# tingyu215/VACNIC

Measured on AMD Instinct MI355X. Metric: train samples/sec, BART-large + CLIP ViT-L/14 full VACNIC step, GoodNews-shaped batch, higher is better.
Workload: dtype bf16

## Files before the change

vacnic_amd/csrc/gemm.hip:

```cpp
#include "gemm_kernel.h"
#include <vector>

using namespace vacgemm;

namespace {

#define VAC_BFLY(ACC, LANE, OFF, HALF)                                                 \
  {                                                                              \
    const bool up = ((LANE) & OFF) != 0;                                           \
    _Pragma("unroll") for (int i = 0; i < HALF; ++i) {                           \
      const float send = up ? ACC[i] : ACC[HALF + i];                            \
      const float keep = up ? ACC[HALF + i] : ACC[i];                            \
      ACC[i] = keep + __shfl_xor(send, OFF, 64);                                 \
    }                                                                            \
  }
#define VAC_BFLY32(ACC, LANE, V, IDX)                                                                                     \
  VAC_BFLY(ACC, LANE, 32, 16) VAC_BFLY(ACC, LANE, 16, 8) VAC_BFLY(ACC, LANE, 8, 4) VAC_BFLY(ACC, LANE, 4, 2) VAC_BFLY(ACC, LANE, 2, 1) \
  float V = ACC[0] + __shfl_xor(ACC[0], 1, 64);                                                                       \
  const int IDX = ((((LANE) >> 5) & 1) << 4) | ((((LANE) >> 4) & 1) << 3) | ((((LANE) >> 3) & 1) << 2) | ((((LANE) >> 2) & 1) << 1) | (((LANE) >> 1) & 1);

template <int MR, int CW, int KW>
__global__ __launch_bounds__(64 * KW) void gemm_skinny_kernel(GemmP p) {
  const int lane = threadIdx.x & 63;
  const int kw = KW == 1 ? 0 : __builtin_amdgcn_readfirstlane(threadIdx.x >> 6);
// ... 208 lines not shown
static const double kFixedUnits = 27e6;

static double cfg_cost(const TileCfg& c, int64_t M, int64_t N, int64_t kper, int64_t z) {
  const int64_t tiles = ((M + c.bm - 1) / c.bm) * ((N + c.bn - 1) / c.bn) * z;
  const int64_t rounds = (tiles + c.slots - 1) / c.slots;
  return (double)rounds * ((double)c.per_cu * c.bm * c.bn * (double)kper / c.eff + kFixedUnits);
}

static int gemm_one(const vacnic_gemm_args* a, int hint, void* stream, int ce_mode = 0, int ce_col0 = 0, bool ce_smooth = false);

static int gemm_env_debug() {
  static int env_debug = -1;
  if (env_debug < 0) { const char* e = getenv("VACNIC_GEMM_DEBUG"); env_debug = e ? atoi(e) : 0; }
  return env_debug;
}

extern "C" int64_t vacnic_gemm_workspace_bytes(int64_t M, int64_t N, int64_t split_k) {
  if (M <= 0 || N <= 0 || split_k <= 1) return 0;
  const int64_t mp = (M + 255) / 256 * 256, np = (N + 255) / 256 * 256;
  return mp * np * 4 * split_k;
}
extern "C" int64_t vacnic_gemm_counters(int64_t M, int64_t N) {
  if (M <= 0 || N <= 0) return 0;
  return ((M + 63) / 64) * ((N + 127) / 128);
}

extern "C" int vacnic_gemm_bf16(const vacnic_gemm_args* a, void* stream) {
  VPLAN_REC_STRUCT(vacnic_gemm_bf16, a, stream);
  VCHECK(a && a->x && a->w && a->out, VACNIC_BAD_SHAPE, "gemm: null operand");
  VCHECK(a->M > 0 && a->N > 0 && a->K > 0, VACNIC_BAD_SHAPE, "gemm: empty problem M=%ld N=%ld K=%ld",
         (long)a->M, (long)a->N, (long)a->K);
  if (a->tile_hint != 0) return gemm_one(a, a->tile_hint, stream);
  if (a->M <= 8 && !a->x_kstrided && !a->w_kstrided && a->split_k <= 1 && !a->preact && !a->dact_src && !a->residual && !a->xsum &&
      (a->K & 7) == 0)
    return gemm_one(a, 8, stream);
  const int split = a->split_k < 1 ? 1 : a->split_k;
  int64_t kper = (a->K + split - 1) / split;
  kper = (kper + BK - 1) / BK * BK;
  const int64_t z = (a->K + kper - 1) / kper;
  int best = 0; double best_cost = 1e300;
  for (int i = 0; i < 3; ++i) {
    if (i == 0 && (a->M < 256 || a->N < 256)) continue;
    const double c = cfg_cost(kCfgs[i], a->M, a->N, kper, z);
    if (c < best_cost) { best_cost = c; best = i; }
  }
  int split_cfg = -1; int64_t m_main = 0; double split_cost = best_cost;
  for (int i = 0; i < 2; ++i) {
    const int64_t rem = a->M % kCfgs[i].bm;
    if (rem == 0 || a->M - rem < kCfgs[i].bm || (i == 0 && a->N < 256)) continue;
    const double c = cfg_cost(kCfgs[i], a->M - rem, a->N, kper, z) + cfg_cost(kCfgs[2], rem, a->N, kper, z);
    if (c < 0.85 * split_cost) { split_cost = c; split_cfg = i; m_main = a->M - rem; }
  }
  const bool fwd8 = !a->x_kstrided && !a->w_kstrided && a->drop_p == 0.f;
  auto loop_of = [&](int hint) { return hint == 256 && fwd8 ? 258 : hint; };
  if (split_cfg < 0) return gemm_one(a, loop_of(kCfgs[best].hint), stream);
  vacnic_gemm_args main_a = *a, tail_a = *a;
  main_a.M = m_main;
  tail_a.M = a->M - m_main;
  const int64_t xoff = a->x_kstrided ? m_main : m_main * a->ldx;
  tail_a.x = (const char*)a->x + xoff * 2;
  const int64_t osz = a->out_mode == 0 ? 2 : 4;
  tail_a.out = (char*)a->out + m_main * a->ldo * osz;
  if (a->preact) tail_a.preact = (char*)a->preact + m_main * a->ldo * 2;
  if (a->dact_src) tail_a.dact_src = (const char*)a->dact_src + m_main * a->ldo * 2;
  if (a->residual) tail_a.residual = (const char*)a->residual + m_main * a->ldo * 2;
  if (a->xsum) tail_a.xsum = a->xsum + m_main;
  if (int e = gemm_one(&main_a, loop_of(kCfgs[split_cfg].hint), stream)) return e;
  return gemm_one(&tail_a, kCfgs[2].hint, stream);
}

static int gemm_one(const vacnic_gemm_args* a, int tile_hint, void* stream, int ce_mode, int ce_col0, bool ce_smooth) {
  VCHECK((a->ldx & 7) == 0 && (a->ldw & 7) == 0, VACNIC_MISALIGNED, "gemm: ldx/ldw must be multiples of 8");
  VCHECK(aligned16(a->x) && aligned16(a->w), VACNIC_MISALIGNED, "gemm: x/w must be 16-byte aligned");
  VCHECK(a->out_mode >= 0 && a->out_mode <= 2, VACNIC_BAD_DTYPE, "gemm: bad out_mode %d", a->out_mode);
  const int split = a->split_k < 1 ? 1 : a->split_k;
  VCHECK(split == 1 || a->out_mode == 2 || a->workspace, VACNIC_UNSUPPORTED, "gemm: split_k needs out_mode 2 or a fix-up workspace");
  if (a->workspace && split > 1) {
    VCHECK(a->counters && aligned16(a->workspace), VACNIC_BAD_SHAPE, "gemm: the split-K fix-up needs `counters` and a 16-byte aligned workspace");
    VCHECK(a->workspace_bytes >= vacnic_gemm_workspace_bytes(a->M, a->N, split) && a->counters_len >= vacnic_gemm_counters(a->M, a->N), VACNIC_BAD_SHAPE,
           "gemm: fix-up workspace %ld B / %ld counters, need %ld B / %ld", (long)a->workspace_bytes, (long)a->counters_len,
           (long)vacnic_gemm_workspace_bytes(a->M, a->N, split), (long)vacnic_gemm_counters(a->M, a->N));
    VCHECK(tile_hint != 8 && !ce_mode, VACNIC_UNSUPPORTED, "gemm: no split-K fix-up in the skinny / cross-entropy kernels");
  }
  VCHECK(a->bias == nullptr || aligned16(a->bias), VACNIC_MISALIGNED, "gemm: bias must be 16-byte aligned");
  VCHECK(a->ldo >= a->N, VACNIC_BAD_SHAPE, "gemm: ldo < N");
  VCHECK(!a->xsum || ce_mode || (a->x_kstrided && a->w_kstrided), VACNIC_UNSUPPORTED,
         "gemm: xsum (row sums of X) is implemented for the weight-gradient layout only (x_kstrided and w_kstrided)");
  if (a->x_kstrided) VCHECK(a->ldx >= ((a->M + 7) & ~7LL), VACNIC_BAD_SHAPE, "gemm: ldx too small for K-strided X");
  else VCHECK(a->ldx >= ((a->K + 7) & ~7LL), VACNIC_BAD_SHAPE, "gemm: ldx < round_up(K, 8) for K-contiguous X");
  if (a->w_kstrided) VCHECK(a->ldw >= ((a->N + 7) & ~7LL), VACNIC_BAD_SHAPE, "gemm: ldw too small for K-strided W");
  else VCHECK(a->ldw >= ((a->K + 7) & ~7LL), VACNIC_BAD_SHAPE, "gemm: ldw < round_up(K, 8) for K-contiguous W");

  auto span = [](int64_t rows, int64_t cols, int64_t ld) { return ((rows - 1) * ld + cols) * 2; };
  const int64_t K8 = (a->K + 7) & ~7LL;
  const int64_t xb = a->x_kstrided ? span(a->K, (a->M + 7) & ~7LL, a->ldx) : span(a->M, K8, a->ldx);
  const int64_t wb = a->w_kstrided ? span(a->K, (a->N + 7) & ~7LL, a->ldw) : span(a->N, K8, a->ldw);
  VCHECK(xb < 0x7ffffff0LL && wb < 0x7ffffff0LL, VACNIC_UNSUPPORTED, "gemm: operand larger than 2 GiB");

  GemmP p;
  p.x = (const bf16_t*)a->x; p.w = (const bf16_t*)a->w; p.bias = a->bias;
  p.out = a->out; p.preact = (bf16_t*)a->preact; p.dact_src = (const bf16_t*)a->dact_src;
  p.residual = (const bf16_t*)a->residual;
  p.xsum = a->xsum;
  p.M = (int)a->M; p.N = (int)a->N; p.K = (int)a->K;
  p.ldx = (int)a->ldx; p.ldw = (int)a->ldw; p.ldo = (int)a->ldo;
  p.act = a->act; p.out_mode = ce_mode ? ce_mode : a->out_mode; p.split_k = split;
  p.ce_col0 = ce_col0;
  int kps = (int)((a->K + split - 1) / split);
  kps = (kps + BK - 1) / BK * BK;
  p.k_per_split = kps;
  const int zsplits = (int)((a->K + kps - 1) / kps);
  p.split_k = zsplits;
  p.alpha = a->alpha;
  p.x_bytes = (unsigned)xb; p.w_bytes = (unsigned)wb;
  p.tiles_m = p.tiles_n = 0;
  p.ws = (a->workspace && zsplits > 1) ? (float*)a->workspace : nullptr;
  p.cnt = p.ws ? a->counters : nullptr;
  p.drop_thr = 0; p.drop_inv = 1.f; p.drop_seed = a->drop_seed; p.drop_seed_dev = (const unsigned long long*)a->drop_seed_dev;
  if (a->drop_p != 0.f) {
    VCHECK(a->drop_p > 0.f && a->drop_p < 1.f, VACNIC_BAD_SHAPE, "gemm: drop_p must be in [0, 1)");
    VCHECK(a->out_mode == 0 && a->ldo == a->N && (a->N & 15) == 0 && !ce_mode && tile_hint != 8, VACNIC_UNSUPPORTED,
           "gemm: fused activation dropout needs a contiguous bf16 output with N %% 16 == 0 (use vacnic_dropout_bf16)");
    VCHECK((zsplits == 1 || p.ws) , VACNIC_UNSUPPORTED, "gemm: fused activation dropout with split-K needs the fix-up workspace");
    unsigned thr = (unsigned)(a->drop_p * 256.f + 0.5f);
    if (thr > 255) thr = 255;
    p.drop_thr = thr;
    p.drop_inv = 256.f / (256.f - (float)thr);
  }
  hipStream_t s = (hipStream_t)stream;
  if (tile_hint == 8) {
    VCHECK(a->M <= 8 && !a->x_kstrided && !a->w_kstrided && zsplits == 1 && !a->preact && !a->dact_src && !a->residual && !a->xsum &&
           (a->K & 7) == 0, VACNIC_UNSUPPORTED, "gemm: the skinny kernel needs M <= 8, K-contiguous operands, K %% 8 == 0 and a plain epilogue");
    constexpr int CW = 4;
    dim3 grid((unsigned)((a->N + CW - 1) / CW));
    if (a->K >= 2048 && a->N <= 8192) hipLaunchKernelGGL((gemm_skinny_kernel<8, CW, 4>), grid, dim3(256), 0, s, p);
    else hipLaunchKernelGGL((gemm_skinny_kernel<8, CW, 1>), grid, dim3(64), 0, s, p);
    VLAUNCH_CHECK();
    return VACNIC_OK;
  }
  const int force = tile_hint % 1000;
  p.debug = tile_hint / 1000 | gemm_env_debug();
  if (((a->M - 1) * a->ldo + a->N) * 2 >= 0x7ffffff0LL) p.debug |= EPI_F32_STAGED;
  if ((a->preact != nullptr) + (a->dact_src != nullptr) + (a->residual != nullptr) > 1) p.debug |= EPI_F32_STAGED;
  if (p.drop_thr && !a->preact && !a->dact_src) p.debug |= EPI_F32_STAGED;
  const bool big = force == 256;
  const bool mid = force == 128;
  if (p.drop_thr) {
    if (big) return launch_t256d(p, a->x_kstrided, a->w_kstrided, zsplits, s);
    if (force == 264) return launch_t264d(p, a->x_kstrided, a->w_kstrided, zsplits, s);
    return launch_t64d(p, a->x_kstrided, a->w_kstrided, zsplits, s);
  }
  if (force == 260) return launch_t260(p, a->x_kstrided, a->w_kstrided, zsplits, s);
  if (force == 261) return launch_t261(p, a->x_kstrided, a->w_kstrided, zsplits, s);
  if (force == 262) return launch_t262(p, a->x_kstrided, a->w_kstrided, zsplits, s);
  if (force == 264) return launch_t264(p, a->x_kstrided, a->w_kstrided, zsplits, s);
  if (force == 258 && !ce_mode) return launch_t258(p, a->x_kstrided, a->w_kstrided, zsplits, s);
  if (ce_mode && ce_smooth) return launch_t256cels(p, a->x_kstrided, a->w_kstrided, zsplits, s);
  if (ce_mode) return launch_t256ce(p, a->x_kstrided, a->w_kstrided, zsplits, s);
  if (big) return launch_t256(p, a->x_kstrided, a->w_kstrided, zsplits, s);
  if (mid) return launch_t128(p, a->x_kstrided, a->w_kstrided, zsplits, s);
  return launch_t64(p, a->x_kstrided, a->w_kstrided, zsplits, s);
}

extern "C" int vacnic_wgrad_group(const vacnic_wgrad_job* jobs, int64_t njobs, void* stream) {
  VCHECK(jobs && njobs > 0, VACNIC_BAD_SHAPE, "wgrad_group: no jobs");
  vplan::Guard vplan_guard__;
  if (vplan::outermost()) {
    std::vector<vacnic_wgrad_job> copy__(jobs, jobs + njobs);
    vplan::push([copy__, stream]() { return vacnic_wgrad_group(copy__.data(), (int64_t)copy__.size(), stream); });
  }
  constexpr int64_t US = (int64_t)GROUP_UT * 128;
  GroupP g;
  g.nunits = 0;
  g.debug = gemm_env_debug() & ~DBG_RETURN;
  auto flush = [&]() -> int {
    if (g.nunits == 0) return VACNIC_OK;
    int kmax = 0;
    for (int i = 0; i < g.nunits; ++i) kmax = g.u[i].K > kmax ? g.u[i].K : kmax;
    g.k_per_phase = (kmax + BK - 1) / BK * BK;
    g.kphase = 0;
    const int e = launch_group128(g, (hipStream_t)stream);
    g.nunits = 0;
    return e;
  };
  auto span = [](int64_t rows, int64_t cols, int64_t ld) { return ((rows - 1) * ld + cols) * 2; };
  for (int64_t j = 0; j < njobs; ++j) {
    const vacnic_wgrad_job& a = jobs[j];
    VCHECK(a.dy && a.x && a.dw, VACNIC_BAD_SHAPE, "wgrad_group: job %ld has a null operand", (long)j);
    VCHECK(a.M > 0 && a.N > 0 && a.K > 0, VACNIC_BAD_SHAPE, "wgrad_group: job %ld is empty (M=%ld N=%ld K=%ld)", (long)j, (long)a.M, (long)a.N, (long)a.K);
    VCHECK((a.lddy & 7) == 0 && (a.ldx & 7) == 0 && aligned16(a.dy) && aligned16(a.x), VACNIC_MISALIGNED,
           "wgrad_group: job %ld: dy / x rows must be 16-byte aligned (ld %% 8 == 0)", (long)j);
    VCHECK(a.lddy >= ((a.N + 7) & ~7LL) && a.ldx >= ((a.K + 7) & ~7LL) && a.lddw >= a.K, VACNIC_BAD_SHAPE,
           "wgrad_group: job %ld: leading dimension too small", (long)j);
    VCHECK((a.lddw & 3) == 0 && aligned16(a.dw), VACNIC_MISALIGNED, "wgrad_group: job %ld: dw rows must be 16-byte aligned", (long)j);
    const int64_t xb = span(a.M, (a.N + 7) & ~7LL, a.lddy), wb = span(a.M, (a.K + 7) & ~7LL, a.ldx);
    VCHECK(xb < 0x7ffffff0LL && wb < 0x7ffffff0LL, VACNIC_UNSUPPORTED, "wgrad_group: job %ld: operand larger than 2 GiB", (long)j);
    for (int64_t um0 = 0; um0 < a.N; um0 += US)
      for (int64_t un0 = 0; un0 < a.K; un0 += US) {
        GroupUnit& u = g.u[g.nunits++];
// ... 175 lines not shown
```

vacnic_amd/csrc/gemm_kernel.h:

```cpp
#pragma once
#include "common.h"
#include <stdlib.h>

namespace vacgemm {


constexpr int BK = 64;
constexpr int OOB = 0x7ffffff0;

struct GemmP {
  const bf16_t* x; const bf16_t* w; const float* bias;
  void* out; bf16_t* preact; const bf16_t* dact_src; const bf16_t* residual;
  float* xsum;
  int M, N, K;
  int ldx, ldw, ldo;
  int act, out_mode, split_k, k_per_split;
  float alpha;
  unsigned x_bytes, w_bytes;
  int tiles_m, tiles_n;
  int ce_col0;
  unsigned drop_thr; float drop_inv; unsigned long long drop_seed; const unsigned long long* drop_seed_dev;
  float* ws;
  unsigned* cnt;
  int debug;
// ... 159 lines not shown
#pragma unroll
    for (int j = 0; j < 8; ++j) v[j] *= act_bwd(p.act, d[j]);
  } else if (p.act != VACNIC_ACT_NONE) {
#pragma unroll
    for (int j = 0; j < 8; ++j) v[j] = act_fwd(p.act, v[j]);
  }
  if (p.residual) {
    float d[8] = {0, 0, 0, 0, 0, 0, 0, 0};
    if (vec) load8bf(p.residual + off, d);
    else for (int j = 0; j < nv; ++j) d[j] = bf2f(p.residual[off + j]);
#pragma unroll
    for (int j = 0; j < 8; ++j) v[j] += d[j];
  }
  if (p.debug & DBG_NO_STORE) {
    if (v[0] == 12345.678f) ((bf16_t*)p.out)[off] = 0;
  } else if (p.out_mode == 0) {
    bf16_t* o = (bf16_t*)p.out + off;
    if (vec) store8bf(o, v);
    else for (int j = 0; j < nv; ++j) o[j] = f2bf(v[j]);
  } else if (p.out_mode == 1) {
    float* o = (float*)p.out + off;
    if (nv == 8 && (p.ldo & 3) == 0) {
      *(f32x4*)o = (f32x4){v[0], v[1], v[2], v[3]};
      *(f32x4*)(o + 4) = (f32x4){v[4], v[5], v[6], v[7]};
    } else {
      for (int j = 0; j < nv; ++j) o[j] = v[j];
    }
  } else {
    float* o = (float*)p.out + off;
    if (nv == 8 && (p.ldo & 3) == 0) {
      f32x4 a0 = *(f32x4*)o, a1 = *(f32x4*)(o + 4);
#pragma unroll
      for (int j = 0; j < 4; ++j) { a0[j] += v[j]; a1[j] += v[4 + j]; }
      *(f32x4*)o = a0; *(f32x4*)(o + 4) = a1;
    } else {
      for (int j = 0; j < nv; ++j) o[j] += v[j];
    }
  }
}

template <int V> struct IC { static constexpr int value = V; };

__device__ __forceinline__ void lds_barrier() {
  asm volatile("s_waitcnt lgkmcnt(0)" ::: "memory");
  __builtin_amdgcn_s_barrier();
  asm volatile("" ::: "memory");
}



template <int N>
__device__ __forceinline__ void wait_vm_lgkm() { asm volatile("s_waitcnt vmcnt(%0) lgkmcnt(0)" ::"n"(N) : "memory"); }

template <int FB, int FA>
__device__ __forceinline__ void p8_loop(f32x4 (&acc)[FB][FA], char* smem, __amdgpu_buffer_rsrc_t xs, __amdgpu_buffer_rsrc_t ws,
                                        int m0, int n0, int RX, int RW, int kbeg, int kend, int ntile, int ldx, int ldw,
                                        int wave, int lane) {
  static_assert(FB == 4 && FA == 8, "128 x 64 outputs per wave");
  constexpr int HALF = 16384, BUF = 4 * HALF;
  constexpr int SLOT_W0 = 0, SLOT_X0 = HALF, SLOT_W1 = 2 * HALF, SLOT_X1 = 3 * HALF;
  const int wm = wave & 1, wn = wave >> 1;
  const int sr = lane >> 2, sc = (lane & 3) ^ (((lane >> 5) & 1) << 1);
  unsigned xoff[2], woff[2];
#pragma unroll
  for (int h = 0; h < 2; ++h) {
    const int gx = m0 + (wave >> 2) * 128 + h * 64 + (wave & 3) * 16 + sr;
    const int gw = n0 + (wave >> 1) * 64 + h * 32 + (wave & 1) * 16 + sr;
    xoff[h] = gx < RX ? ((unsigned)gx * (unsigned)ldx + (unsigned)(sc * 8)) * 2u : (unsigned)OOB;
    woff[h] = gw < RW ? ((unsigned)gw * (unsigned)ldw + (unsigned)(sc * 8)) * 2u : (unsigned)OOB;
  }
  const int klim = kend - sc * 8;
  char* const sdst = smem + wave * 2048;
  auto stage = [&](__amdgpu_buffer_rsrc_t rsrc, unsigned roff, int slot, int t) {
    const int k0 = kbeg + t * 64;
    const unsigned v0 = k0 < klim ? roff + (unsigned)k0 * 2u : (unsigned)OOB;
    const unsigned v1 = k0 + 32 < klim ? roff + (unsigned)(k0 + 32) * 2u : (unsigned)OOB;
    char* d = sdst + slot;
    __builtin_amdgcn_raw_ptr_buffer_load_lds(rsrc, LDS_PTR(d), 16, (int)v0, 0, 0, 0);
    __builtin_amdgcn_raw_ptr_buffer_load_lds(rsrc, LDS_PTR(d + 1024), 16, (int)v1, 0, 0, 0);
  };
  const int fro = (lane & 15) * 64 + (((lane >> 4) ^ (((lane >> 3) & 1) << 1)) << 4);
  const char* const xrd = smem + fro + wm * 8192;
  const char* const wrd = smem + fro + wn * 4096;

  stage(ws, woff[0], SLOT_W0, 0); stage(xs, xoff[0], SLOT_X0, 0); stage(ws, woff[1], SLOT_W1, 0); stage(xs, xoff[1], SLOT_X1, 0);
  stage(ws, woff[0], BUF + SLOT_W0, 1); stage(xs, xoff[0], BUF + SLOT_X0, 1); stage(ws, woff[1], BUF + SLOT_W1, 1);
  asm volatile("s_waitcnt vmcnt(6)" ::: "memory");
  __builtin_amdgcn_sched_barrier(0);
  __builtin_amdgcn_s_barrier();
  __builtin_amdgcn_sched_barrier(0);
  const bool grp_b = wave >= 4;
  if (grp_b) { __builtin_amdgcn_sched_barrier(0); __builtin_amdgcn_s_barrier(); __builtin_amdgcn_sched_barrier(0); }

  bf16x8 xf[4][2], w0[2][2], w1[2][2];
#define VAC_P8_BAR()  __builtin_amdgcn_sched_barrier(0); __builtin_amdgcn_s_barrier(); __builtin_amdgcn_sched_barrier(0)
#define VAC_P8_MFMA(A0, B0, WF)                                                                                          \
  asm volatile("s_waitcnt lgkmcnt(0)" ::: "memory");                                                                     \
  __builtin_amdgcn_sched_barrier(0);                                                                                     \
  __builtin_amdgcn_s_setprio(1);                                                                                         \
  _Pragma("unroll") for (int kk = 0; kk < 2; ++kk)                                                                       \
    _Pragma("unroll") for (int b = 0; b < 2; ++b)                                                                        \
      _Pragma("unroll") for (int a = 0; a < 4; ++a)                                                                      \
        acc[B0 + b][A0 + a] = __builtin_amdgcn_mfma_f32_16x16x32_bf16(WF[b][kk], xf[a][kk], acc[B0 + b][A0 + a], 0, 0, 0); \
  __builtin_amdgcn_s_setprio(0);                                                                                         \
  VAC_P8_BAR()
  auto ktile = [&](auto par_c, int t) {
    constexpr int PAR = decltype(par_c)::value;
    const char* const xb = xrd + PAR * BUF;
    const char* const wb = wrd + PAR * BUF;
#pragma unroll
    for (int b = 0; b < 2; ++b)
#pragma unroll
      for (int kk = 0; kk < 2; ++kk) w0[b][kk] = *(const bf16x8*)(wb + SLOT_W0 + b * 2048 + kk * 1024);
    __builtin_amdgcn_sched_barrier(0);
// ... 52 lines not shown
  const int kend = min(p.K, kbeg + p.k_per_split);
  const int ntile = (p.debug & DBG_NO_KLOOP) ? 0 : (kend - kbeg + BKT - 1) / BKT;

  __amdgpu_buffer_rsrc_t xs = __builtin_amdgcn_make_buffer_rsrc((void*)p.x, 0, p.x_bytes, 0x00020000);
  __amdgpu_buffer_rsrc_t ws = __builtin_amdgcn_make_buffer_rsrc((void*)p.w, 0, p.w_bytes, 0x00020000);

  const int RX = XKS ? ((p.M + 7) & ~7) : p.M;
  const int RW = WKS ? ((p.N + 7) & ~7) : p.N;

  f32x4 acc[FB][FA];
#pragma unroll
  for (int b = 0; b < FB; ++b)
#pragma unroll
    for (int a = 0; a < FA; ++a) acc[b][a] = (f32x4){0.f, 0.f, 0.f, 0.f};

  constexpr int XSN = FA / WN;
  static_assert(FA % WN == 0 && FA / WN <= 4, "xsum: row blocks split over the waves of a row group, <= 4 each");
  constexpr bool XS = XKS && WKS;
  const bool xs_on = XS && p.xsum != nullptr;
  int xs_next = tn;
  f32x4 accs = (f32x4){0.f, 0.f, 0.f, 0.f};
#define VAC_XSUM_MFMA(XF)                                                                   \
  if constexpr (XS) {                                                                       \
    _Pragma("unroll") for (int w_ = 0; w_ < WN; ++w_)                                       \
      if (wn == w_) {                                                                       \
        _Pragma("unroll") for (int i = 0; i < XSN; ++i) {                                   \
          const short o_ = (lane & 15) == i ? (short)0x3F80 : (short)0;                              \
          const bf16x8 sel_ = {o_, o_, o_, o_, o_, o_, o_, o_};                             \
          accs = __builtin_amdgcn_mfma_f32_16x16x32_bf16(sel_, XF[w_ * XSN + i], accs, 0, 0, 0); \
        }                                                                                   \
      }                                                                                     \
  }
#define VAC_XSUM(XF, STEP)                                                                  \
  if (XS && xs_on && (STEP) == xs_next) {                                                   \
    VAC_XSUM_MFMA(XF)                                                                       \
    xs_next += p.tiles_n;                                                                   \
  }

  constexpr int LOADS = (BM + BN) * BKT * 2 / 1024 / NWAVE;
  static_assert(LOADS * (NSTAGE - 2) <= 63, "vmcnt immediate");
  constexpr bool PIPED = PIPE && BKT == 64 && NSTAGE == 2 && !P8;
  constexpr int PRO = PIPED ? 2 : NSTAGE - 1;
  if constexpr (!P8) {
#pragma unroll
    for (int s = 0; s < PRO; ++s) {
      stage_tile<XKS, BM, BKT, NWAVE>(xs, smem + s * STAGE, m0, RX, kbeg + s * BKT, kend, p.ldx, wave, lane);
      stage_tile<WKS, BN, BKT, NWAVE>(ws, smem + s * STAGE + XT, n0, RW, kbeg + s * BKT, kend, p.ldw, wave, lane);
    }
    wait_vm_lgkm<LOADS * (PRO - 1)>();
    __builtin_amdgcn_s_barrier();
  }
  int cur = 0, nxt = NSTAGE - 1;
  if constexpr (P8) {
    static_assert(BM == 256 && BN == 256 && WM == 2 && WN == 4 && BKT == 64 && NSTAGE == 2 && !XKS && !WKS,
                  "8-phase loop: 256 x 256 tile, 2 x 4 waves, both operands K-contiguous");
    p8_loop(acc, smem, xs, ws, m0, n0, RX, RW, kbeg, kend, ntile, p.ldx, p.ldw, wave, lane);
  } else if constexpr (PIPE && BKT == 32 && NSTAGE == 4) {
    static_assert(NWAVE == 8 && LOADS >= 2, "ping-pong loop is written for 8 waves (two per SIMD)");
    const bool grp_b = wave >= NWAVE / 2;
    const int nst = ntile;
    bf16x8 xf[FA], wf[FB];
    if (grp_b) { __builtin_amdgcn_sched_barrier(0); __builtin_amdgcn_s_barrier(); __builtin_amdgcn_sched_barrier(0); }
    int rd = 0, wr = 3;
    for (int h = 0; h < nst; ++h) {
      const char* xr = smem + rd * STAGE;
      char* xw = smem + wr * STAGE;
      if (!(p.debug & DBG_NO_FRAG_READS) || h == 0) {
#pragma unroll
        for (int a = 0; a < FA; ++a) xf[a] = read_frag<XKS, BM, BKT>(xr, wm * TM + a * 16, 0, lane);
#pragma unroll
        for (int b = 0; b < FB; ++b) wf[b] = read_frag<WKS, BN, BKT>(xr + XT, wn * TN + b * 16, 0, lane);
      }
      if (!(p.debug & DBG_NO_DMA)) {
        stage_tile<XKS, BM, BKT, NWAVE>(xs, xw, m0, RX, kbeg + (h + 3) * BKT, kend, p.ldx, wave, lane);
        stage_tile<WKS, BN, BKT, NWAVE>(ws, xw + XT, n0, RW, kbeg + (h + 3) * BKT, kend, p.ldw, wave, lane);
      }
      wait_vm_lgkm<2 * LOADS>();
      __builtin_amdgcn_sched_barrier(0);
      __builtin_amdgcn_s_barrier();
      __builtin_amdgcn_sched_barrier(0);
      __builtin_amdgcn_s_setprio(1);
#pragma unroll
      for (int b = 0; b < FB; ++b)
#pragma unroll
        for (int a = 0; a < FA; ++a)
          acc[b][a] = __builtin_amdgcn_mfma_f32_16x16x32_bf16(wf[b], xf[a], acc[b][a], 0, 0, 0);
      VAC_XSUM(xf, h)
      __builtin_amdgcn_s_setprio(0);
      __builtin_amdgcn_sched_barrier(0);
      __builtin_amdgcn_s_barrier();
      __builtin_amdgcn_sched_barrier(0);
      rd = (rd + 1) & 3;
      wr = (wr + 1) & 3;
    }
    if (!grp_b) { __builtin_amdgcn_sched_barrier(0); __builtin_amdgcn_s_barrier(); __builtin_amdgcn_sched_barrier(0); }
  } else if constexpr (PIPED) {
    bf16x8 xf0[FA], wf0[FB], xf1[FA], wf1[FB];
#pragma unroll
    for (int a = 0; a < FA; ++a) xf0[a] = read_frag<XKS, BM, BKT>(smem, wm * TM + a * 16, 0, lane);
#pragma unroll
    for (int b = 0; b < FB; ++b) wf0[b] = read_frag<WKS, BN, BKT>(smem + XT, wn * TN + b * 16, 0, lane);
    for (int t = 0; t < ntile; ++t) {
      char* xcur = smem + cur * STAGE;
      char* wcur = xcur + XT;
#pragma unroll
      for (int a = 0; a < FA; ++a) xf1[a] = read_frag<XKS, BM, BKT>(xcur, wm * TM + a * 16, 1, lane);
#pragma unroll
      for (int b = 0; b < FB; ++b) wf1[b] = read_frag<WKS, BN, BKT>(wcur, wn * TN + b * 16, 1, lane);
#pragma unroll
// ... 506 lines not shown
template <int BM, int BN, int WM, int WN, int BKT, int NSTAGE, bool PIPE>
__global__ __launch_bounds__(64 * WM * WN, 2) void gemm_group_kernel(GroupP g) {
  constexpr int TPU = GROUP_UT * GROUP_UT;
  const int xcd = blockIdx.x & 7, j = blockIdx.x >> 3;
  const int unit = (j / TPU) * 8 + xcd;
  if (unit >= g.nunits) return;
  const int t = j % TPU;
  const int tm = t / GROUP_UT, tn = t % GROUP_UT;
  const GroupUnit& u = g.u[unit];
  const int m0 = u.um0 + tm * BM, n0 = u.un0 + tn * BN;
  if (m0 >= u.M || n0 >= u.N || g.kphase * g.k_per_phase >= u.K) return;
  GemmP p;
  p.x = u.x; p.w = u.w; p.bias = nullptr; p.out = u.out; p.preact = nullptr; p.dact_src = nullptr; p.residual = nullptr;
  p.xsum = u.xsum;
  p.M = u.M; p.N = u.N; p.K = u.K; p.ldx = u.ldx; p.ldw = u.ldw; p.ldo = u.ldo;
  p.act = VACNIC_ACT_NONE; p.out_mode = 2; p.split_k = 1; p.k_per_split = g.k_per_phase;
  p.alpha = 1.0f; p.x_bytes = u.x_bytes; p.w_bytes = u.w_bytes;
  p.tiles_m = GROUP_UT; p.tiles_n = min(GROUP_UT, (u.N - u.un0 + BN - 1) / BN);
  p.ce_col0 = 0; p.debug = g.debug; p.ws = nullptr; p.cnt = nullptr; p.drop_thr = 0;
  gemm_tile<BM, BN, WM, WN, BKT, NSTAGE, PIPE, true, true, false>(p, m0, n0, tn, g.kphase);
}

template <auto KERN, size_t LDS, class P>
void launch_lds(dim3 grid, dim3 block, hipStream_t s, const P& p) {
  if (LDS > 65536) {
    static bool once = false;
    if (!once) { (void)hipFuncSetAttribute((const void*)KERN, hipFuncAttributeMaxDynamicSharedMemorySize, (int)LDS); once = true; }
  }
  hipLaunchKernelGGL(KERN, grid, block, LDS, s, p);
}

template <int BM, int BN, int WM, int WN, int BKT, int NSTAGE, bool PIPE>
int launch_gemm_ce_smooth(const GemmP& p0, bool xks, bool wks, int zsplits, hipStream_t s) {
  if (xks || wks || zsplits != 1) { vacnic_set_error("gemm: the cross-entropy epilogues are built for the forward layout without split-K"); return VACNIC_UNSUPPORTED; }
  GemmP p = p0;
  p.tiles_m = (p.M + BM - 1) / BM; p.tiles_n = (p.N + BN - 1) / BN;
  constexpr size_t lds = NSTAGE * (BM + BN) * BKT * 2;
  static_assert(lds >= 64 * (BN + 4) * 4, "epilogue staging must fit in the operand buffers");
  launch_lds<gemm_ce_smooth_kernel<BM, BN, WM, WN, BKT, NSTAGE, PIPE>, lds>(dim3(p.tiles_m * p.tiles_n), dim3(64 * WM * WN), s, p);
  VLAUNCH_CHECK();
  return VACNIC_OK;
}

template <int BM, int BN, int WM, int WN, int BKT, int NSTAGE, bool PIPE>
int launch_gemm_group(const GroupP& g, hipStream_t s) {
  static_assert(BM == 128 && BN == 128, "units are GROUP_UT x GROUP_UT tiles of 128 x 128");
  const int rounds = (g.nunits + 7) / 8;
  constexpr size_t lds = NSTAGE * (BM + BN) * BKT * 2;
  launch_lds<gemm_group_kernel<BM, BN, WM, WN, BKT, NSTAGE, PIPE>, lds>(dim3(rounds * 8 * GROUP_UT * GROUP_UT), dim3(64 * WM * WN), s, g);
  VLAUNCH_CHECK();
  return VACNIC_OK;
}

template <int BM, int BN, int WM, int WN, int BKT, int NSTAGE, bool PIPE = false, bool CE = false, bool DR = false, bool P8 = false>
int launch_gemm(const GemmP& p0, bool xks, bool wks, int zsplits, hipStream_t s) {
  GemmP p = p0;
  p.tiles_m = (p.M + BM - 1) / BM; p.tiles_n = (p.N + BN - 1) / BN;
  const dim3 grid(p.tiles_m * p.tiles_n * zsplits), block(64 * WM * WN);
  constexpr size_t lds = NSTAGE * (BM + BN) * BKT * 2;
  static_assert(lds >= 64 * (BN + 4) * 4, "epilogue staging must fit in the operand buffers");
  auto launch = [&](auto xk, auto wk) {
    launch_lds<gemm_kernel<BM, BN, WM, WN, BKT, NSTAGE, PIPE, decltype(xk)::value != 0, decltype(wk)::value != 0, CE, DR, P8>, lds>(grid, block, s, p);
  };
  constexpr IC<0> no{};
  constexpr IC<1> yes{};
  if constexpr (P8) {
    if (xks || wks) { vacnic_set_error("gemm: the 8-phase loop is built for the forward layout (both operands K-contiguous)"); return VACNIC_UNSUPPORTED; }
    launch(no, no);
  } else if constexpr (CE) {
    if (xks || wks) { vacnic_set_error("gemm: the cross-entropy epilogues are built for the forward layout only"); return VACNIC_UNSUPPORTED; }
    launch(no, no);
  } else if constexpr (DR) {
    if (xks) { vacnic_set_error("gemm: fused activation dropout is built for K-contiguous X (forward / dgrad layouts)"); return VACNIC_UNSUPPORTED; }
    if (wks) launch(no, yes); else launch(no, no);
  } else {
    if (!xks && !wks) launch(no, no);
    else if (!xks && wks) launch(no, yes);
    else if (xks && wks) launch(yes, yes);
    else launch(yes, no);
  }
  VLAUNCH_CHECK();
  return VACNIC_OK;
}


int launch_t256(const GemmP& p, bool xks, bool wks, int zsplits, hipStream_t s);
int launch_t258(const GemmP& p, bool xks, bool wks, int zsplits, hipStream_t s);
int launch_t264(const GemmP& p, bool xks, bool wks, int zsplits, hipStream_t s);
int launch_t128(const GemmP& p, bool xks, bool wks, int zsplits, hipStream_t s);
int launch_t64(const GemmP& p, bool xks, bool wks, int zsplits, hipStream_t s);
int launch_t260(const GemmP& p, bool xks, bool wks, int zsplits, hipStream_t s);
int launch_t261(const GemmP& p, bool xks, bool wks, int zsplits, hipStream_t s);
int launch_t262(const GemmP& p, bool xks, bool wks, int zsplits, hipStream_t s);
int launch_t256ce(const GemmP& p, bool xks, bool wks, int zsplits, hipStream_t s);
int launch_t256cels(const GemmP& p, bool xks, bool wks, int zsplits, hipStream_t s);
int launch_t256d(const GemmP& p, bool xks, bool wks, int zsplits, hipStream_t s);
int launch_t264d(const GemmP& p, bool xks, bool wks, int zsplits, hipStream_t s);
int launch_t64d(const GemmP& p, bool xks, bool wks, int zsplits, hipStream_t s);
int launch_group128(const GroupP& g, hipStream_t s);

}
```

vacnic_amd/ops.py:

```python
import contextlib

import torch
from torch.autograd import Function

from . import ddp
from . import kernels as K
from . import streams

BF16 = torch.bfloat16


class Rng:
    base = 0x5EED
    counter = 0

    @classmethod
    def manual_seed(cls, s):
        cls.base = int(s) & 0xFFFFFFFF
        cls.counter = 0

    @classmethod
    def next(cls):
        cls.counter += 1
        return (cls.base << 32) | (cls.counter & 0xFFFFFFFF)
# ... 122 lines not shown
        for M in list(self.by_m):
            self._launch(M)

    def reset(self):
        self.by_m.clear()
        self.units.clear()
        self.dst.clear()
        self.armed = False


_WGQ = _WgradQueue()


def flush_wgrads():
    _WGQ.flush()


def begin_step():
    _WGQ.reset()
    if streams.pending_keep():
        streams.join_all()


def _groupable(dy2d, x2d, spec, M):
    return (WGRAD_GROUP and spec.wgrad is not None and WGRAD_GROUP_MIN_M <= M <= WGRAD_GROUP_MAX_M and spec.N >= 512 and spec.K >= 512
            and dy2d.stride(0) % 8 == 0 and x2d.stride(0) % 8 == 0 and spec.wgrad.stride(0) % 4 == 0
            and dy2d.shape[1] == spec.N and x2d.shape[1] == spec.K)


def _wgrad(dy2d, x2d, spec, M):
    side = streams.raw("wgrad")
    if side is not None:
        K.fence(K._stream(), side)
    if _groupable(dy2d, x2d, spec, M):
        _WGQ.add(dy2d, x2d, spec, M)
        return
    with _on_wgrad():
        _wgrad_impl(dy2d, x2d, spec, M)
    ddp.done(spec.wgrad, spec.bgrad)


def _wgrad_impl(dy2d, x2d, spec, M):
    if spec.wgrad is None:
        if spec.bgrad is not None:
            K.bias_grad(dy2d, spec.bgrad, M, spec.N)
        return
    N, Kd = spec.N, spec.K
    tiles = ((N + 127) // 128) * ((Kd + 127) // 128)
    split = K.wgrad_split(M, tiles)
    if split > 1 and M >= 4096:
        hint = 128
        if N >= 512 and Kd >= 512:
            hint, split = (128, 8) if N * Kd <= (1 << 20) else (256, 4)
        K.gemm(dy2d, x2d, N, Kd, M, out=spec.wgrad, ldx=dy2d.stride(0), ldw=x2d.stride(0), ldo=spec.wgrad.stride(0),
               x_kstrided=True, w_kstrided=True, out_mode=2, split_k=split, xsum=spec.bgrad, fixup=True, tile_hint=hint)
        return
    K.gemm(dy2d, x2d, N, Kd, M, out=spec.wgrad, ldx=dy2d.stride(0), ldw=x2d.stride(0), ldo=spec.wgrad.stride(0),
           x_kstrided=True, w_kstrided=True, out_mode=2, split_k=split, xsum=spec.bgrad)


class LinearFn(Function):

    @staticmethod
    def forward(ctx, x, anchor, spec, residual, ge, skip):
        _tag(ctx)
        Kd = spec.K
        x2 = _c(x).view(-1, Kd)
        M = x2.shape[0]
        out = torch.empty(x.shape[:-1] + (spec.N,), device=x.device, dtype=BF16)
        K.gemm(x2, spec.w16, M, spec.N, Kd, bias=spec.bias, out=out, ldw=spec.ldw,
               residual=_c(residual) if residual is not None else None)
        ctx.spec, ctx.M = spec, M
        ctx.has_res = residual is not None
        ctx.save_for_backward(x2)
        ddp.expect(ge and any(ctx.needs_input_grad), spec.wgrad, spec.bgrad)
        if skip:
            return out, x.view_as(x)
        return out

    @_bw
    def backward(ctx, dy, dskip=None):
        (x2,) = ctx.saved_tensors
        spec, M = ctx.spec, ctx.M
        if dy is None:
            ddp.done(spec.wgrad, spec.bgrad)
            return dskip, None, None, None, None, None
        dy2 = _c(dy).view(M, spec.N)
        dx = None
        if ctx.needs_input_grad[0]:
            dx = torch.empty((M, spec.K), device=dy.device, dtype=BF16)
            K.gemm(dy2, spec.w16, M, spec.K, spec.N, out=dx, ldw=spec.ldw, w_kstrided=True,
                   residual=_c(dskip).view(M, spec.K) if dskip is not None else None)
            dx = dx.view(dy.shape[:-1] + (spec.K,))
        _wgrad(dy2, x2, spec, M)
        return dx, None, None, (dy if ctx.has_res else None), None, None


def linear(x, anchor, spec, residual=None):
    return LinearFn.apply(x, anchor, spec, residual, torch.is_grad_enabled(), False)


def linear_skip(x, anchor, spec):
    if not (torch.is_grad_enabled() and x.requires_grad):
        return linear(x, anchor, spec), x
    return LinearFn.apply(x, anchor, spec, None, True, True)

# ... 489 lines not shown
```

Measured before the change: 491.9.

## Extend 8-phase 256x256 GEMM loop to dgrad and weight-gradient K-strided layouts

Generalizes the 8-phase ping-pong p8_loop so it also handles K-strided W (dgrad) and K-strided X and W (weight gradient). It uses transposing LDS reads (ds_read_b64_tr_b16) and folds the bias-gradient column sums into extra MFMAs. New hint 259 kernels are dispatched automatically for 256-tile backward GEMMs when the grid is small enough, and the Python weight-gradient path selects them too. This is meant to give backward GEMMs the better-overlapped schedule that forward already had. It adds two more template instantiations and new swizzle and offset logic that carries correctness risk.

New measurement: 493.2, median of 6. No clear change (+0.3%).

```diff
diff --git a/vacnic_amd/csrc/gemm.hip b/vacnic_amd/csrc/gemm.hip
--- a/vacnic_amd/csrc/gemm.hip
+++ b/vacnic_amd/csrc/gemm.hip
@@ -284,8 +284,13 @@
     if (c < 0.85 * split_cost) { split_cost = c; split_cfg = i; m_main = a->M - rem; }
   }
   const bool fwd8 = !a->x_kstrided && !a->w_kstrided && a->drop_p == 0.f;
-  auto loop_of = [&](int hint) { return hint == 256 && fwd8 ? 258 : hint; };
-  if (split_cfg < 0) return gemm_one(a, loop_of(kCfgs[best].hint), stream);
+  auto strided8 = [&](int64_t m) {
+    if (!a->w_kstrided || a->drop_p != 0.f) return false;
+    if (!a->x_kstrided) return true;
+    return z == 1 || ((m + 255) / 256) * ((a->N + 255) / 256) * z < 256;
+  };
+  auto loop_of = [&](int hint, int64_t m) { return hint != 256 ? hint : fwd8 ? 258 : strided8(m) ? 259 : hint; };
+  if (split_cfg < 0) return gemm_one(a, loop_of(kCfgs[best].hint, a->M), stream);
   vacnic_gemm_args main_a = *a, tail_a = *a;
   main_a.M = m_main;
   tail_a.M = a->M - m_main;
@@ -297,7 +302,7 @@
   if (a->dact_src) tail_a.dact_src = (const char*)a->dact_src + m_main * a->ldo * 2;
   if (a->residual) tail_a.residual = (const char*)a->residual + m_main * a->ldo * 2;
   if (a->xsum) tail_a.xsum = a->xsum + m_main;
-  if (int e = gemm_one(&main_a, loop_of(kCfgs[split_cfg].hint), stream)) return e;
+  if (int e = gemm_one(&main_a, loop_of(kCfgs[split_cfg].hint, m_main), stream)) return e;
   return gemm_one(&tail_a, kCfgs[2].hint, stream);
 }
 
@@ -377,6 +382,11 @@
   if (p.drop_thr && !a->preact && !a->dact_src) p.debug |= EPI_F32_STAGED;
   const bool big = force == 256;
   const bool mid = force == 128;
+  if (force == 259) {
+    VCHECK(!ce_mode && !p.drop_thr, VACNIC_UNSUPPORTED, "gemm: tile hint 259 has no cross-entropy / fused-dropout epilogues (those stay on the ping-pong kernels)");
+    VCHECK(a->w_kstrided, VACNIC_UNSUPPORTED, "gemm: tile hint 259 is the 8-phase loop for K-strided W (dgrad, weight gradient); the forward layout is hint 258");
+    return a->x_kstrided ? launch_t259w(p, true, true, zsplits, s) : launch_t259d(p, false, true, zsplits, s);
+  }
   if (p.drop_thr) {
     if (big) return launch_t256d(p, a->x_kstrided, a->w_kstrided, zsplits, s);
     if (force == 264) return launch_t264d(p, a->x_kstrided, a->w_kstrided, zsplits, s);
diff --git a/vacnic_amd/csrc/gemm_kernel.h b/vacnic_amd/csrc/gemm_kernel.h
--- a/vacnic_amd/csrc/gemm_kernel.h
+++ b/vacnic_amd/csrc/gemm_kernel.h
@@ -235,14 +235,167 @@
 template <int N>
 __device__ __forceinline__ void wait_vm_lgkm() { asm volatile("s_waitcnt vmcnt(%0) lgkmcnt(0)" ::"n"(N) : "memory"); }
 
-template <int FB, int FA>
+template <int FB, int FA, bool XKS = false, bool WKS = false>
 __device__ __forceinline__ void p8_loop(f32x4 (&acc)[FB][FA], char* smem, __amdgpu_buffer_rsrc_t xs, __amdgpu_buffer_rsrc_t ws,
                                         int m0, int n0, int RX, int RW, int kbeg, int kend, int ntile, int ldx, int ldw,
-                                        int wave, int lane) {
+                                        int wave, int lane, f32x4& accs, bool xs_on, int& xs_next, int tiles_n) {
   static_assert(FB == 4 && FA == 8, "128 x 64 outputs per wave");
+  static_assert(WKS || !XKS, "K-strided X comes with K-strided W only (the weight-gradient layout)");
   constexpr int HALF = 16384, BUF = 4 * HALF;
   constexpr int SLOT_W0 = 0, SLOT_X0 = HALF, SLOT_W1 = 2 * HALF, SLOT_X1 = 3 * HALF;
   const int wm = wave & 1, wn = wave >> 1;
+  if constexpr (XKS || WKS) {
+    const int kl = wave * 8 + (lane >> 4);
+    const int slc = (lane & 15) ^ ((((lane >> 4) & 3) | ((wave & 1) << 2)) << 1);
+    const int sr = lane >> 2, sc = (lane & 3) ^ (((lane >> 5) & 1) << 1);
+    unsigned xoff[2], woff[2];
+#pragma unroll
+    for (int h = 0; h < 2; ++h) {
+      if constexpr (XKS) {
+        const int gx = m0 + (slc >> 3) * 128 + h * 64 + (slc & 7) * 8;
+        xoff[h] = gx < RX ? (unsigned)gx * 2u : (unsigned)OOB;
+      } else {
+        const int gx = m0 + (wave >> 2) * 128 + h * 64 + (wave & 3) * 16 + sr;
+        xoff[h] = gx < RX ? ((unsigned)gx * (unsigned)ldx + (unsigned)(sc * 8)) * 2u : (unsigned)OOB;
+      }
+      const int gw = n0 + (slc >> 2) * 64 + h * 32 + (slc & 3) * 8;
+      woff[h] = gw < RW ? (unsigned)gw * 2u : (unsigned)OOB;
+    }
+    const int klim = kend - sc * 8;
+    char* const sdst = smem + wave * 2048;
+    auto stage_kc = [&](__amdgpu_buffer_rsrc_t rsrc, unsigned roff, int slot, int t) {
+      const int k0 = kbeg + t * 64;
+      const unsigned v0 = k0 < klim ? roff + (unsigned)k0 * 2u : (unsigned)OOB;
+      const unsigned v1 = k0 + 32 < klim ? roff + (unsigned)(k0 + 32) * 2u : (unsigned)OOB;
+      char* d = sdst + slot;
+      __builtin_amdgcn_raw_ptr_buffer_load_lds(rsrc, LDS_PTR(d), 16, (int)v0, 0, 0, 0);
+      __builtin_amdgcn_raw_ptr_buffer_load_lds(rsrc, LDS_PTR(d + 1024), 16, (int)v1, 0, 0, 0);
+    };
+    auto stage_ks = [&](__amdgpu_buffer_rsrc_t rsrc, unsigned roff, int slot, int t, int ld) {
+      const int k0 = kbeg + t * 64 + kl;
+      const unsigned v0 = k0 < kend ? roff + (unsigned)k0 * (unsigned)ld * 2u : (unsigned)OOB;
+      const unsigned v1 = k0 + 4 < kend ? roff + (unsigned)(k0 + 4) * (unsigned)ld * 2u : (unsigned)OOB;
+      char* d = sdst + slot;
+      __builtin_amdgcn_raw_ptr_buffer_load_lds(rsrc, LDS_PTR(d), 16, (int)v0, 0, 0, 0);
+      __builtin_amdgcn_raw_ptr_buffer_load_lds(rsrc, LDS_PTR(d + 1024), 16, (int)v1, 0, 0, 0);
+    };
+    auto stage_x = [&](int h, int slot, int t) {
+      if constexpr (XKS) stage_ks(xs, xoff[h], slot, t, ldx); else stage_kc(xs, xoff[h], slot, t);
+    };
+    auto stage_w = [&](int h, int slot, int t) { stage_ks(ws, woff[h], slot, t, ldw); };
+    const int g = lane >> 4, q = (lane & 15) >> 2, pp = lane & 3;
+    const int rsw = (q | ((g & 1) << 2)) << 1;
+    const int kro = (8 * g + q) * 256 + (pp & 1) * 8;
+    const int fro = (lane & 15) * 64 + (((lane >> 4) ^ (((lane >> 3) & 1) << 1)) << 4);
+    int xra[4], wra[2];
+#pragma unroll
+    for (int a = 0; a < 4; ++a) xra[a] = XKS ? kro + (((wm * 8 + a * 2 + (pp >> 1)) ^ rsw) << 4) : fro + wm * 8192 + a * 2048;
+#pragma unroll
+    for (int b = 0; b < 2; ++b) wra[b] = kro + (((wn * 4 + b * 2 + (pp >> 1)) ^ rsw) << 4);
+    auto tr8 = [&](auto off_c, unsigned a) {
+      constexpr int OFF = decltype(off_c)::value;
+      static_assert(OFF >= 0 && OFF + 1024 < 65536, "ds offset field");
+      bf16x4 t0, t1;
+      asm volatile("ds_read_b64_tr_b16 %0, %1 offset:%2" : "=v"(t0) : "v"(a), "n"(OFF) : "memory");
+      asm volatile("ds_read_b64_tr_b16 %0, %1 offset:%2" : "=v"(t1) : "v"(a), "n"(OFF + 1024) : "memory");
+      return __builtin_shufflevector(t0, t1, 0, 1, 2, 3, 4, 5, 6, 7);
+    };
+    const unsigned sbase = (unsigned)(size_t)LDS_PTR(smem);
+    auto read_x = [&](auto par_c, auto slot_c, auto kk_c, int a) {
+      constexpr int PAR = decltype(par_c)::value, SLOT = decltype(slot_c)::value, KK = decltype(kk_c)::value;
+      if constexpr (XKS) return tr8(IC<SLOT + KK * 8192>{}, sbase + (unsigned)(PAR * BUF) + (unsigned)xra[a]);
+      else return *(const bf16x8*)(smem + PAR * BUF + SLOT + xra[a] + KK * 1024);
+    };
+    auto read_w = [&](auto par_c, auto slot_c, auto kk_c, int b) {
+      constexpr int PAR = decltype(par_c)::value, SLOT = decltype(slot_c)::value, KK = decltype(kk_c)::value;
+      return tr8(IC<SLOT + KK * 8192>{}, sbase + (unsigned)(PAR * BUF) + (unsigned)wra[b]);
+    };
+    constexpr int NXA = XKS ? 4 : 2;
+
+    stage_w(0, SLOT_W0, 0); stage_x(0, SLOT_X0, 0); stage_w(1, SLOT_W1, 0); stage_x(1, SLOT_X1, 0);
+    stage_w(0, BUF + SLOT_W0, 1); stage_x(0, BUF + SLOT_X0, 1); stage_w(1, BUF + SLOT_W1, 1);
+    asm volatile("s_waitcnt vmcnt(6)" ::: "memory");
+    __builtin_amdgcn_sched_barrier(0);
+    __builtin_amdgcn_s_barrier();
+    __builtin_amdgcn_sched_barrier(0);
+    const bool grp_b = wave >= 4;
+    if (grp_b) { __builtin_amdgcn_sched_barrier(0); __builtin_amdgcn_s_barrier(); __builtin_amdgcn_sched_barrier(0); }
+
+    bf16x8 xf[4][2], w0[2][2], w1[2][2];
+    auto xsum_half = [&](auto h_c, int t) {
+      if constexpr (XKS && WKS) {
+        constexpr int H = decltype(h_c)::value;
+        if (xs_on && (wn >> 1) == H) {
+#pragma unroll
+          for (int kk = 0; kk < 2; ++kk)
+            if (2 * t + kk == xs_next) {
+#pragma unroll
+              for (int i = 0; i < 2; ++i) {
+                const short o_ = (lane & 15) == i ? (short)0x3F80 : (short)0;
+                const bf16x8 sel_ = {o_, o_, o_, o_, o_, o_, o_, o_};
+                if (wn & 1) accs = __builtin_amdgcn_mfma_f32_16x16x32_bf16(sel_, xf[2 + i][kk], accs, 0, 0, 0);
+                else accs = __builtin_amdgcn_mfma_f32_16x16x32_bf16(sel_, xf[i][kk], accs, 0, 0, 0);
+              }
+              xs_next += tiles_n;
+            }
+        }
+      }
+    };
+#define VAC_P8_BAR()  __builtin_amdgcn_sched_barrier(0); __builtin_amdgcn_s_barrier(); __builtin_amdgcn_sched_barrier(0)
+#define VAC_P8_MFMA(A0, B0, WF, TAIL)                                                                                    \
+  asm volatile("s_waitcnt lgkmcnt(0)" ::: "memory");                                                                     \
+  __builtin_amdgcn_sched_barrier(0);                                                                                     \
+  __builtin_amdgcn_s_setprio(1);                                                                                         \
+  _Pragma("unroll") for (int kk = 0; kk < 2; ++kk)                                                                       \
+    _Pragma("unroll") for (int b = 0; b < 2; ++b)                                                                        \
+      _Pragma("unroll") for (int a = 0; a < 4; ++a)                                                                      \
+        acc[B0 + b][A0 + a] = __builtin_amdgcn_mfma_f32_16x16x32_bf16(WF[b][kk], xf[a][kk], acc[B0 + b][A0 + a], 0, 0, 0); \
+  TAIL;                                                                                                                  \
+  __builtin_amdgcn_s_setprio(0);                                                                                         \
+  VAC_P8_BAR()
+    auto ktile = [&](auto par_c, int t) {
+      constexpr int PAR = decltype(par_c)::value;
+      constexpr IC<0> k0{};
+      constexpr IC<1> k1{};
+#pragma unroll
+      for (int b = 0; b < 2; ++b) { w0[b][0] = read_w(par_c, IC<SLOT_W0>{}, k0, b); w0[b][1] = read_w(par_c, IC<SLOT_W0>{}, k1, b); }
+      __builtin_amdgcn_sched_barrier(0);
+      xf[0][0] = read_x(par_c, IC<SLOT_X0>{}, k0, 0); xf[0][1] = read_x(par_c, IC<SLOT_X0>{}, k1, 0);
+      __builtin_amdgcn_sched_barrier(0);
+      stage_x(1, (PAR ^ 1) * BUF + SLOT_X1, t + 1);
+      asm volatile("s_waitcnt lgkmcnt(%0)" ::"n"(NXA) : "memory");
+      __builtin_amdgcn_sched_barrier(0);
+#pragma unroll
+      for (int a = 1; a < 4; ++a) { xf[a][0] = read_x(par_c, IC<SLOT_X0>{}, k0, a); xf[a][1] = read_x(par_c, IC<SLOT_X0>{}, k1, a); }
+      VAC_P8_BAR();
+      VAC_P8_MFMA(0, 0, w0, xsum_half(IC<0>{}, t));
+#pragma unroll
+      for (int b = 0; b < 2; ++b) { w1[b][0] = read_w(par_c, IC<SLOT_W1>{}, k0, b); w1[b][1] = read_w(par_c, IC<SLOT_W1>{}, k1, b); }
+      __builtin_amdgcn_sched_barrier(0);
+      stage_w(0, PAR * BUF + SLOT_W0, t + 2);
+      VAC_P8_BAR();
+      VAC_P8_MFMA(0, 2, w1, (void)0);
+#pragma unroll
+      for (int a = 0; a < 4; ++a) { xf[a][0] = read_x(par_c, IC<SLOT_X1>{}, k0, a); xf[a][1] = read_x(par_c, IC<SLOT_X1>{}, k1, a); }
+      __builtin_amdgcn_sched_barrier(0);
+      stage_x(0, PAR * BUF + SLOT_X0, t + 2);
+      VAC_P8_BAR();
+      VAC_P8_MFMA(4, 2, w1, xsum_half(IC<1>{}, t));
+      stage_w(1, PAR * BUF + SLOT_W1, t + 2);
+      asm volatile("s_waitcnt vmcnt(6)" ::: "memory");
+      VAC_P8_BAR();
+      VAC_P8_MFMA(4, 0, w0, (void)0);
+    };
+    for (int t = 0; t < ntile; t += 2) {
+      ktile(IC<0>{}, t);
+      if (t + 1 >= ntile) break;
+      ktile(IC<1>{}, t + 1);
+    }
+#undef VAC_P8_MFMA
+#undef VAC_P8_BAR
+    if (!grp_b) { __builtin_amdgcn_sched_barrier(0); __builtin_amdgcn_s_barrier(); __builtin_amdgcn_sched_barrier(0); }
+    return;
+  }
   const int sr = lane >> 2, sc = (lane & 3) ^ (((lane >> 5) & 1) << 1);
   unsigned xoff[2], woff[2];
 #pragma unroll
@@ -401,9 +554,9 @@
   }
   int cur = 0, nxt = NSTAGE - 1;
   if constexpr (P8) {
-    static_assert(BM == 256 && BN == 256 && WM == 2 && WN == 4 && BKT == 64 && NSTAGE == 2 && !XKS && !WKS,
-                  "8-phase loop: 256 x 256 tile, 2 x 4 waves, both operands K-contiguous");
-    p8_loop(acc, smem, xs, ws, m0, n0, RX, RW, kbeg, kend, ntile, p.ldx, p.ldw, wave, lane);
+    static_assert(BM == 256 && BN == 256 && WM == 2 && WN == 4 && BKT == 64 && NSTAGE == 2 && (WKS || !XKS),
+                  "8-phase loop: 256 x 256 tile, 2 x 4 waves; forward, dgrad (W K-strided) and weight-gradient (both K-strided) layouts");
+    p8_loop<FB, FA, XKS, WKS>(acc, smem, xs, ws, m0, n0, RX, RW, kbeg, kend, ntile, p.ldx, p.ldw, wave, lane, accs, xs_on, xs_next, p.tiles_n);
   } else if constexpr (PIPE && BKT == 32 && NSTAGE == 4) {
     static_assert(NWAVE == 8 && LOADS >= 2, "ping-pong loop is written for 8 waves (two per SIMD)");
     const bool grp_b = wave >= NWAVE / 2;
@@ -1016,7 +1169,7 @@
   return VACNIC_OK;
 }
 
-template <int BM, int BN, int WM, int WN, int BKT, int NSTAGE, bool PIPE = false, bool CE = false, bool DR = false, bool P8 = false>
+template <int BM, int BN, int WM, int WN, int BKT, int NSTAGE, bool PIPE = false, bool CE = false, bool DR = false, bool P8 = false, int P8KS = 0>
 int launch_gemm(const GemmP& p0, bool xks, bool wks, int zsplits, hipStream_t s) {
   GemmP p = p0;
   p.tiles_m = (p.M + BM - 1) / BM; p.tiles_n = (p.N + BN - 1) / BN;
@@ -1028,7 +1181,13 @@
   };
   constexpr IC<0> no{};
   constexpr IC<1> yes{};
-  if constexpr (P8) {
+  if constexpr (P8 && P8KS == 1) {
+    if (xks || !wks) { vacnic_set_error("gemm: this 8-phase kernel is built for the dgrad layout (W K-strided, X K-contiguous)"); return VACNIC_UNSUPPORTED; }
+    launch(no, yes);
+  } else if constexpr (P8 && P8KS == 2) {
+    if (!xks || !wks) { vacnic_set_error("gemm: this 8-phase kernel is built for the weight-gradient layout (X and W K-strided)"); return VACNIC_UNSUPPORTED; }
+    launch(yes, yes);
+  } else if constexpr (P8) {
     if (xks || wks) { vacnic_set_error("gemm: the 8-phase loop is built for the forward layout (both operands K-contiguous)"); return VACNIC_UNSUPPORTED; }
     launch(no, no);
   } else if constexpr (CE) {
@@ -1050,6 +1209,8 @@
 
 int launch_t256(const GemmP& p, bool xks, bool wks, int zsplits, hipStream_t s);
 int launch_t258(const GemmP& p, bool xks, bool wks, int zsplits, hipStream_t s);
+int launch_t259d(const GemmP& p, bool xks, bool wks, int zsplits, hipStream_t s);
+int launch_t259w(const GemmP& p, bool xks, bool wks, int zsplits, hipStream_t s);
 int launch_t264(const GemmP& p, bool xks, bool wks, int zsplits, hipStream_t s);
 int launch_t128(const GemmP& p, bool xks, bool wks, int zsplits, hipStream_t s);
 int launch_t64(const GemmP& p, bool xks, bool wks, int zsplits, hipStream_t s);
diff --git a/vacnic_amd/csrc/gemm_t259.hip b/vacnic_amd/csrc/gemm_t259.hip
--- /dev/null
+++ b/vacnic_amd/csrc/gemm_t259.hip
@@ -0,0 +1,4 @@
+#include "gemm_kernel.h"
+namespace vacgemm {
+int launch_t259d(const GemmP& p, bool xks, bool wks, int zsplits, hipStream_t s) { return launch_gemm<256, 256, 2, 4, 64, 2, false, false, false, true, 1>(p, xks, wks, zsplits, s); }
+}
diff --git a/vacnic_amd/csrc/gemm_t259w.hip b/vacnic_amd/csrc/gemm_t259w.hip
--- /dev/null
+++ b/vacnic_amd/csrc/gemm_t259w.hip
@@ -0,0 +1,4 @@
+#include "gemm_kernel.h"
+namespace vacgemm {
+int launch_t259w(const GemmP& p, bool xks, bool wks, int zsplits, hipStream_t s) { return launch_gemm<256, 256, 2, 4, 64, 2, false, false, false, true, 2>(p, xks, wks, zsplits, s); }
+}
diff --git a/vacnic_amd/ops.py b/vacnic_amd/ops.py
--- a/vacnic_amd/ops.py
+++ b/vacnic_amd/ops.py
@@ -198,6 +198,8 @@
         hint = 128
         if N >= 512 and Kd >= 512:
             hint, split = (128, 8) if N * Kd <= (1 << 20) else (256, 4)
+            if hint == 256 and ((N + 255) // 256) * ((Kd + 255) // 256) * split < 256:
+                hint = 259
         K.gemm(dy2d, x2d, N, Kd, M, out=spec.wgrad, ldx=dy2d.stride(0), ldw=x2d.stride(0), ldo=spec.wgrad.stride(0),
                x_kstrided=True, w_kstrided=True, out_mode=2, split_k=split, xsum=spec.bgrad, fixup=True, tile_hint=hint)
         return
```
